# Stoffel-Labs/mpc-protocols

Hardware: AMD Instinct MI355X
Metric: shares/sec (compute_shares) + recons/sec (batch_recon), 256-bit Fr, 1/2/4/8 GPU (higher is better)
Workload: dtype u32; 1 GPU; compute_shares n=16 t=5 batch=2^20 secrets per GPU (BASELINE configs[1]); field=bls12-381 Fr, parallelism=batch-sharded x1, no data-path collective, field_impl=u29

## Files before the change

mpc-protocols_amd/csrc/kernels_mfma_bfly_ring.hpp:

```cpp
#pragma once
#include "bfly_ring_plan.hpp"
#include "kernels_mfma_bfly.hpp"

namespace hbmpc {
namespace mf {

HB_DEV void ring_dma16(const uint8_t* sbase, uint32_t voff, uint32_t lds_dst) {
    uint32_t keep;
    asm volatile("s_mov_b32 %0, m0\n\ts_mov_b32 m0, %3\n\ts_nop 4\n\tglobal_load_lds_dwordx4 %1, %2\n\ts_mov_b32 m0, %0"
                 : "=&s"(keep)
                 : "v"(voff), "s"(sbase), "s"(lds_dst)
                 : "memory");
}
using ring_flag_t = __attribute__((address_space(3))) volatile uint32_t;
HB_DEV uint32_t ring_flag(const ring_flag_t* p) { return __builtin_amdgcn_readfirstlane(*p); }

template <int M, int CW, int NP, int S, int D>
__global__ __launch_bounds__(64 * (CW + 1)) void k_mfma_bfly_ring(MfmaRowsArgs a) {
    static_assert(bfly_ring_shape_ok(M, NP, BflyRingShape{CW, S, D}), "ring shape");
    static_assert(M * (D - 1) <= 63, "vmcnt counts to 63");
    constexpr int ROWB = M * 1024 + MF_BFLY_BIAS;
    constexpr int NT = 64 * (CW + 1);
    constexpr int TILEB = M * 1024;
    extern __shared__ __attribute__((aligned(16))) uint8_t lds[];
    const int blk8 = (int)blockIdx.x >> 3;
    const uint32_t wg_in_role = (uint32_t)a.blk_idx[blk8] * 8 + (blockIdx.x & 7);
    const MfmaRole role = a.role[0];
    const uint32_t role_wgs = (uint32_t)a.role_nwg[0];
    bfly_table_to_lds<NT>(lds, a.table + (size_t)role.row0 * ROWB, NP * (ROWB / 16));
    uint8_t* const ring = lds + bfly_ring_table_bytes(M, NP);
    ring_flag_t* const filled = (ring_flag_t*)(lds + bfly_ring_flags_offset(M, NP, S));
    ring_flag_t* const freed = filled + S;
    if (threadIdx.x < 2 * S) filled[threadIdx.x] = 0;
    __syncthreads();
    const uint32_t lane = threadIdx.x & 63, wave = __builtin_amdgcn_readfirstlane(threadIdx.x >> 6);
    const uint32_t nitems = (uint32_t)bfly_ring_items(bfly_ring_ntiles(a.G), role_wgs, wg_in_role, CW);
    auto tile_of = [&](uint32_t q) { return bfly_ring_tile(role_wgs, wg_in_role, CW, q); };
    if (wave == CW) {
        if (nitems == 0) return;
        const size_t total = a.G * (size_t)(M * 32);
        auto wait_freed = [&](uint32_t q) {
            if (q >= S) {
                const uint32_t need = q / S;
                while (ring_flag(freed + q % S) != need) __builtin_amdgcn_s_sleep(1);
            }
        };
        auto publish = [&](uint32_t q) { filled[q % S] = q / S + 1; };
        auto piece = [&](size_t tb, int i) {
            const uint32_t off = (uint32_t)(i * 64 + lane) * 16u;
            const size_t left = total - tb;
            return left >= (size_t)TILEB || off + 16 <= left ? off : (uint32_t)(left - 16);
        };
        const uint32_t ring_lds = (uint32_t)(uintptr_t)ring;
        for (uint32_t q = 0; q < nitems; ++q) {
            wait_freed(q);
            const size_t tb = tile_of(q) * (size_t)(32 * M * 32);
            const uint32_t dst = __builtin_amdgcn_readfirstlane(ring_lds + (q % S) * TILEB);
#pragma unroll
            for (int i = 0; i < M; ++i) ring_dma16(a.in + tb, piece(tb, i), dst + i * 1024);
            if (q + 1 >= D) {
                asm volatile("s_waitcnt vmcnt(%0)" ::"n"(M * (D - 1)) : "memory");
                publish(q + 1 - D);
            }
        }
        asm volatile("s_waitcnt vmcnt(0)" ::: "memory");
        for (uint32_t q = nitems >= D - 1 ? nitems - (D - 1) : 0; q < nitems; ++q) publish(q);
        return;
    }
    const int c = lane & 31, h = lane >> 5;
    const Half H = make_half(h);
    for (uint32_t q = wave; q < nitems; q += CW) {
        const uint32_t slot = q % S, seq = q / S + 1;
        while (ring_flag(filled + slot) != seq) __builtin_amdgcn_s_sleep(1);
        asm volatile("" ::: "memory");
        v4i data[M];
        {
            const uint8_t* sp = ring + slot * TILEB + c * (M * 32) + 16 * h;
#pragma unroll
            for (int i = 0; i < M; ++i) data[i] = *reinterpret_cast<const v4i*>(sp + i * 32);
        }
        asm volatile("s_waitcnt lgkmcnt(0)" ::: "memory");
        freed[slot] = seq;
#pragma unroll
        for (int i = 0; i < M; ++i) data[i] = flip(data[i]);
        const BflyOut o = bfly_out(a, tile_of(q), c, h);
        auto store_row = [&](uint32_t k, bool exists, const uint32_t (&Rw)[4]) {
            uint8_t* qb = a.out_party_major ? a.out + (size_t)k * a.out_stride * 32 : a.out + (size_t)k * 32;
            if (exists && o.live) *reinterpret_cast<uint4*>(qb + o.qo) = make_uint4(Rw[0], Rw[1], Rw[2], Rw[3]);
        };
#pragma unroll
        for (int p = 0; p < NP; ++p) {
            uint32_t pe[8], pt[8];
            bfly_pair<M>(lds + (size_t)p * ROWB, lane, h, data, pe, pt);
            uint32_t k32 = (uint32_t)(role.row0 + p);
            asm volatile("" : "+s"(k32));
            {
                uint64_t T[4];
                uint32_t Rw[4];
#pragma unroll
                for (int j = 0; j < 4; ++j) T[j] = (uint64_t)(pe[2 * j + 1] + pt[2 * j + 1]) * H.k16 + (pe[2 * j] + pt[2 * j]);
                reduce_words(T, Rw, H);
                store_row(k32, true, Rw);
            }
            const bool partner = (int)k32 + a.half < a.nout;
            if (partner) {
                uint64_t T[4];
                uint32_t Rw[4];
#pragma unroll
                for (int j = 0; j < 4; ++j) T[j] = (uint64_t)(pe[2 * j + 1] - pt[2 * j + 1]) * H.k16 + (pe[2 * j] - pt[2 * j]);
                reduce_words(T, Rw, H);
                store_row(k32 + (uint32_t)a.half, true, Rw);
            }
        }
    }
}

}
}
```

mpc-protocols_amd/csrc/tu_mfma_bfly_ring.hip:

```cpp
#include <utility>

#include "kernels_mfma_bfly_ring.hpp"
#include "launchers.hpp"
namespace hbmpc {
namespace {
template <int M, int NP>
bool launch(const mf::MfmaRowsArgs& a, int device, hipStream_t s) {
    if constexpr (mf::bfly_ring_fits(M, NP)) {
        constexpr mf::BflyRingShape R = mf::BFLY_RING_LIB;
        const size_t lds = mf::bfly_ring_lds_bytes(M, NP, R.slots);
        static std::atomic<bool> attr_set[HBMPC_MAX_DEVICES];
        if (!ensure_dynamic_lds(reinterpret_cast<const void*>(&mf::k_mfma_bfly_ring<M, R.cw, NP, R.slots, R.depth>), attr_set, device, lds)) return false;
        hipLaunchKernelGGL((mf::k_mfma_bfly_ring<M, R.cw, NP, R.slots, R.depth>), dim3((unsigned)mf::mf_grid(a)), dim3(64 * (R.cw + 1)), lds, s, a);
        return true;
    }
    return false;
}
template <int M>
bool one(const mf::MfmaRowsArgs& a, int device, hipStream_t s) {
    if (a.role[0].nrows == 8) return launch<M, 8>(a, device, s);
    if (a.role[0].nrows == 4) return launch<M, 4>(a, device, s);
    return false;
}
template <int LO, int... I>
bool range(int m, const mf::MfmaRowsArgs& a, int device, hipStream_t s, std::integer_sequence<int, I...>) {
    bool hit = false;
    ((m == LO + I ? (hit = one<LO + I>(a, device, s)) : false), ...);
    return hit;
}
}
bool launch_mfma_bfly_ring(int m, const mf::MfmaRowsArgs& a, int device, hipStream_t s) {
    if (!a.in_chunk_major || a.in_b || a.ncoeffs || a.list_rows || a.other_stride || a.nroles != 1 || a.G == 0) return false;
    return range<2>(m, a, device, s, std::make_integer_sequence<int, mf::BFLY_RING_MAX_M - 1>{});
}
}
```

Baseline: 115.8 billion shares/s.

## Overlap ring prologue DMA with table load in butterfly ring kernel

The producer wave now issues its first D tile DMAs before the block barrier, while the compute waves load the twiddle table into LDS with direct global-to-LDS DMA instead of a cooperative copy. The flag init and __syncthreads now follow the table load, and the producer joins via s_barrier. This overlaps kernel startup latency (table load and first tile fetches) instead of serialising them. The block index indirection is dropped, and the launcher now rejects any non-identity blk_idx mapping. The producer no longer exits early when it has no items and always participates in the barrier.

```diff
diff --git a/mpc-protocols_amd/csrc/kernels_mfma_bfly_ring.hpp b/mpc-protocols_amd/csrc/kernels_mfma_bfly_ring.hpp
--- a/mpc-protocols_amd/csrc/kernels_mfma_bfly_ring.hpp
+++ b/mpc-protocols_amd/csrc/kernels_mfma_bfly_ring.hpp
@@ -20,24 +20,18 @@
     static_assert(bfly_ring_shape_ok(M, NP, BflyRingShape{CW, S, D}), "ring shape");
     static_assert(M * (D - 1) <= 63, "vmcnt counts to 63");
     constexpr int ROWB = M * 1024 + MF_BFLY_BIAS;
-    constexpr int NT = 64 * (CW + 1);
     constexpr int TILEB = M * 1024;
     extern __shared__ __attribute__((aligned(16))) uint8_t lds[];
-    const int blk8 = (int)blockIdx.x >> 3;
-    const uint32_t wg_in_role = (uint32_t)a.blk_idx[blk8] * 8 + (blockIdx.x & 7);
+    const uint32_t wg_in_role = blockIdx.x;
     const MfmaRole role = a.role[0];
     const uint32_t role_wgs = (uint32_t)a.role_nwg[0];
-    bfly_table_to_lds<NT>(lds, a.table + (size_t)role.row0 * ROWB, NP * (ROWB / 16));
     uint8_t* const ring = lds + bfly_ring_table_bytes(M, NP);
     ring_flag_t* const filled = (ring_flag_t*)(lds + bfly_ring_flags_offset(M, NP, S));
     ring_flag_t* const freed = filled + S;
-    if (threadIdx.x < 2 * S) filled[threadIdx.x] = 0;
-    __syncthreads();
     const uint32_t lane = threadIdx.x & 63, wave = __builtin_amdgcn_readfirstlane(threadIdx.x >> 6);
     const uint32_t nitems = (uint32_t)bfly_ring_items(bfly_ring_ntiles(a.G), role_wgs, wg_in_role, CW);
     auto tile_of = [&](uint32_t q) { return bfly_ring_tile(role_wgs, wg_in_role, CW, q); };
     if (wave == CW) {
-        if (nitems == 0) return;
         const size_t total = a.G * (size_t)(M * 32);
         auto wait_freed = [&](uint32_t q) {
             if (q >= S) {
@@ -52,21 +46,42 @@
             return left >= (size_t)TILEB || off + 16 <= left ? off : (uint32_t)(left - 16);
         };
         const uint32_t ring_lds = (uint32_t)(uintptr_t)ring;
-        for (uint32_t q = 0; q < nitems; ++q) {
-            wait_freed(q);
+        auto request = [&](uint32_t q) {
             const size_t tb = tile_of(q) * (size_t)(32 * M * 32);
             const uint32_t dst = __builtin_amdgcn_readfirstlane(ring_lds + (q % S) * TILEB);
 #pragma unroll
             for (int i = 0; i < M; ++i) ring_dma16(a.in + tb, piece(tb, i), dst + i * 1024);
-            if (q + 1 >= D) {
-                asm volatile("s_waitcnt vmcnt(%0)" ::"n"(M * (D - 1)) : "memory");
-                publish(q + 1 - D);
+        };
+#pragma unroll
+        for (int q = 0; q < D; ++q)
+            if ((uint32_t)q < nitems) request((uint32_t)q);
+        __builtin_amdgcn_s_barrier();
+        for (uint32_t q = D - 1; q < nitems; ++q) {
+            if (q >= D) {
+                wait_freed(q);
+                request(q);
             }
+            asm volatile("s_waitcnt vmcnt(%0)" ::"n"(M * (D - 1)) : "memory");
+            publish(q + 1 - D);
         }
         asm volatile("s_waitcnt vmcnt(0)" ::: "memory");
         for (uint32_t q = nitems >= D - 1 ? nitems - (D - 1) : 0; q < nitems; ++q) publish(q);
         return;
     }
+    {
+        static_assert(NP * ROWB % 1024 == 0, "the table is whole 1-KB pieces");
+        constexpr int KB = NP * ROWB / 1024;
+        const uint8_t* src = a.table + (size_t)role.row0 * ROWB;
+        const uint32_t lds0 = (uint32_t)(uintptr_t)lds;
+#pragma unroll
+        for (int j = 0; j < (KB + CW - 1) / CW; ++j) {
+            const uint32_t k = wave + (uint32_t)j * CW;
+            if (k < (uint32_t)KB) ring_dma16(src + (size_t)k * 1024, lane * 16u, __builtin_amdgcn_readfirstlane(lds0 + k * 1024));
+        }
+        asm volatile("s_waitcnt vmcnt(0)" ::: "memory");
+    }
+    if (threadIdx.x < 2 * S) filled[threadIdx.x] = 0;
+    __syncthreads();
     const int c = lane & 31, h = lane >> 5;
     const Half H = make_half(h);
     for (uint32_t q = wave; q < nitems; q += CW) {
diff --git a/mpc-protocols_amd/csrc/tu_mfma_bfly_ring.hip b/mpc-protocols_amd/csrc/tu_mfma_bfly_ring.hip
--- a/mpc-protocols_amd/csrc/tu_mfma_bfly_ring.hip
+++ b/mpc-protocols_amd/csrc/tu_mfma_bfly_ring.hip
@@ -31,6 +31,8 @@
 }
 bool launch_mfma_bfly_ring(int m, const mf::MfmaRowsArgs& a, int device, hipStream_t s) {
     if (!a.in_chunk_major || a.in_b || a.ncoeffs || a.list_rows || a.other_stride || a.nroles != 1 || a.G == 0) return false;
+    for (int j = 0; j < a.nblocks; ++j)
+        if (a.blk_idx[j] != j) return false;
     return range<2>(m, a, device, s, std::make_integer_sequence<int, mf::BFLY_RING_MAX_M - 1>{});
 }
 }
```

After: 116.8 billion shares/s, median of 6. About the same (+0.9%).

## Prefetch ring tiles before table load and use nontemporal output stores

Applied to the files above, without the earlier changes.

The loader wave now issues its first D tile DMAs before the block-wide barrier, so input fetch overlaps the coefficient table copy into LDS. Only the compute waves load the table, and they stage it through registers. The blk_idx byte is now read as a 32-bit word. Output stores switch to global_store_dwordx4 with the nt modifier by default, so the write-once share stream avoids polluting the cache. The risks are more complex barrier ordering (the loader returns only after the sync) and possible nt store penalties.

```diff
diff --git a/mpc-protocols_amd/csrc/kernels_mfma_bfly_ring.hpp b/mpc-protocols_amd/csrc/kernels_mfma_bfly_ring.hpp
--- a/mpc-protocols_amd/csrc/kernels_mfma_bfly_ring.hpp
+++ b/mpc-protocols_amd/csrc/kernels_mfma_bfly_ring.hpp
@@ -1,44 +1,72 @@
 #pragma once
+#include <stddef.h>
+
 #include "bfly_ring_plan.hpp"
 #include "kernels_mfma_bfly.hpp"
 
 namespace hbmpc {
 namespace mf {
 
+enum RingPolicy { RP_DEFAULT = 0, RP_NT = 1, RP_SC1 = 2, RP_SC0_SC1 = 3 };
+#define HBMPC_RING_DMA16(MOD)                                                                                                       \
+    asm volatile("s_mov_b32 %0, m0\n\ts_mov_b32 m0, %3\n\ts_nop 4\n\tglobal_load_lds_dwordx4 %1, %2" MOD "\n\ts_mov_b32 m0, %0" \
+                 : "=&s"(keep)                                                                                                      \
+                 : "v"(voff), "s"(sbase), "s"(lds_dst)                                                                              \
+                 : "memory")
+template <int POL = RP_DEFAULT>
 HB_DEV void ring_dma16(const uint8_t* sbase, uint32_t voff, uint32_t lds_dst) {
+    static_assert(POL == RP_DEFAULT || POL == RP_NT, "loader policy");
     uint32_t keep;
-    asm volatile("s_mov_b32 %0, m0\n\ts_mov_b32 m0, %3\n\ts_nop 4\n\tglobal_load_lds_dwordx4 %1, %2\n\ts_mov_b32 m0, %0"
-                 : "=&s"(keep)
-                 : "v"(voff), "s"(sbase), "s"(lds_dst)
-                 : "memory");
+    if constexpr (POL == RP_NT) HBMPC_RING_DMA16(" nt");
+    else HBMPC_RING_DMA16("");
 }
+#undef HBMPC_RING_DMA16
+template <int POL>
+HB_DEV void ring_store16(uint8_t* p, const uint32_t (&w)[4]) {
+    static_assert(POL == RP_NT || POL == RP_SC1 || POL == RP_SC0_SC1, "store policy");
+    const v4i v = {(int)w[0], (int)w[1], (int)w[2], (int)w[3]};
+    if constexpr (POL == RP_NT) asm volatile("global_store_dwordx4 %0, %1, off nt" ::"v"(p), "v"(v) : "memory");
+    else if constexpr (POL == RP_SC1) asm volatile("global_store_dwordx4 %0, %1, off sc1" ::"v"(p), "v"(v) : "memory");
+    else asm volatile("global_store_dwordx4 %0, %1, off sc0 sc1" ::"v"(p), "v"(v) : "memory");
+}
+constexpr int BFLY_RING_LOAD_POLICY = RP_DEFAULT, BFLY_RING_STORE_POLICY = RP_NT;
 using ring_flag_t = __attribute__((address_space(3))) volatile uint32_t;
 HB_DEV uint32_t ring_flag(const ring_flag_t* p) { return __builtin_amdgcn_readfirstlane(*p); }
 
-template <int M, int CW, int NP, int S, int D>
+template <int M, int CW, int NP, int S, int D, int LP = BFLY_RING_LOAD_POLICY, int SP = BFLY_RING_STORE_POLICY>
 __global__ __launch_bounds__(64 * (CW + 1)) void k_mfma_bfly_ring(MfmaRowsArgs a) {
     static_assert(bfly_ring_shape_ok(M, NP, BflyRingShape{CW, S, D}), "ring shape");
     static_assert(M * (D - 1) <= 63, "vmcnt counts to 63");
     constexpr int ROWB = M * 1024 + MF_BFLY_BIAS;
-    constexpr int NT = 64 * (CW + 1);
     constexpr int TILEB = M * 1024;
     extern __shared__ __attribute__((aligned(16))) uint8_t lds[];
     const int blk8 = (int)blockIdx.x >> 3;
-    const uint32_t wg_in_role = (uint32_t)a.blk_idx[blk8] * 8 + (blockIdx.x & 7);
+    static_assert(offsetof(MfmaRowsArgs, blk_idx) % 4 == 0, "blk_idx is read by words");
+    const uint32_t blk_word = reinterpret_cast<const uint32_t*>(a.blk_idx)[blk8 >> 2];
+    const uint32_t wg_in_role = ((blk_word >> (8 * (blk8 & 3))) & 0xffu) * 8 + (blockIdx.x & 7);
     const MfmaRole role = a.role[0];
     const uint32_t role_wgs = (uint32_t)a.role_nwg[0];
-    bfly_table_to_lds<NT>(lds, a.table + (size_t)role.row0 * ROWB, NP * (ROWB / 16));
     uint8_t* const ring = lds + bfly_ring_table_bytes(M, NP);
     ring_flag_t* const filled = (ring_flag_t*)(lds + bfly_ring_flags_offset(M, NP, S));
     ring_flag_t* const freed = filled + S;
-    if (threadIdx.x < 2 * S) filled[threadIdx.x] = 0;
-    __syncthreads();
     const uint32_t lane = threadIdx.x & 63, wave = __builtin_amdgcn_readfirstlane(threadIdx.x >> 6);
-    const uint32_t nitems = (uint32_t)bfly_ring_items(bfly_ring_ntiles(a.G), role_wgs, wg_in_role, CW);
+    auto items = [&] { return (uint32_t)bfly_ring_items(bfly_ring_ntiles(a.G), role_wgs, wg_in_role, CW); };
     auto tile_of = [&](uint32_t q) { return bfly_ring_tile(role_wgs, wg_in_role, CW, q); };
     if (wave == CW) {
-        if (nitems == 0) return;
+        const uint32_t nitems = items();
         const size_t total = a.G * (size_t)(M * 32);
+        auto piece = [&](size_t tb, int i) {
+            const uint32_t off = (uint32_t)(i * 64 + lane) * 16u;
+            const size_t left = total - tb;
+            return left >= (size_t)TILEB || off + 16 <= left ? off : (uint32_t)(left - 16);
+        };
+        const uint32_t ring_lds = (uint32_t)(uintptr_t)ring;
+        auto request = [&](uint32_t q) {
+            const size_t tb = tile_of(q) * (size_t)(32 * M * 32);
+            const uint32_t dst = __builtin_amdgcn_readfirstlane(ring_lds + (q % S) * TILEB);
+#pragma unroll
+            for (int i = 0; i < M; ++i) ring_dma16<LP>(a.in + tb, piece(tb, i), dst + i * 1024);
+        };
         auto wait_freed = [&](uint32_t q) {
             if (q >= S) {
                 const uint32_t need = q / S;
@@ -46,22 +74,18 @@
             }
         };
         auto publish = [&](uint32_t q) { filled[q % S] = q / S + 1; };
-        auto piece = [&](size_t tb, int i) {
-            const uint32_t off = (uint32_t)(i * 64 + lane) * 16u;
-            const size_t left = total - tb;
-            return left >= (size_t)TILEB || off + 16 <= left ? off : (uint32_t)(left - 16);
-        };
-        const uint32_t ring_lds = (uint32_t)(uintptr_t)ring;
-        for (uint32_t q = 0; q < nitems; ++q) {
+        for (uint32_t q = 0; q < nitems && q < (uint32_t)D; ++q) request(q);
+        __syncthreads();
+        if (nitems == 0) return;
+        if (nitems >= (uint32_t)D) {
+            asm volatile("s_waitcnt vmcnt(%0)" ::"n"(M * (D - 1)) : "memory");
+            publish(0);
+        }
+        for (uint32_t q = D; q < nitems; ++q) {
             wait_freed(q);
-            const size_t tb = tile_of(q) * (size_t)(32 * M * 32);
-            const uint32_t dst = __builtin_amdgcn_readfirstlane(ring_lds + (q % S) * TILEB);
-#pragma unroll
-            for (int i = 0; i < M; ++i) ring_dma16(a.in + tb, piece(tb, i), dst + i * 1024);
-            if (q + 1 >= D) {
-                asm volatile("s_waitcnt vmcnt(%0)" ::"n"(M * (D - 1)) : "memory");
-                publish(q + 1 - D);
-            }
+            request(q);
+            asm volatile("s_waitcnt vmcnt(%0)" ::"n"(M * (D - 1)) : "memory");
+            publish(q + 1 - D);
         }
         asm volatile("s_waitcnt vmcnt(0)" ::: "memory");
         for (uint32_t q = nitems >= D - 1 ? nitems - (D - 1) : 0; q < nitems; ++q) publish(q);
@@ -69,6 +93,27 @@
     }
     const int c = lane & 31, h = lane >> 5;
     const Half H = make_half(h);
+    uint32_t nitems;
+    {
+        constexpr int PIECES = NP * (ROWB / 16), NTC = 64 * CW, ROUNDS = (PIECES + NTC - 1) / NTC;
+        const uint8_t* src = a.table + (size_t)role.row0 * ROWB;
+        v4i t[ROUNDS];
+#pragma unroll
+        for (int k = 0; k < ROUNDS; ++k) {
+            const int p = (int)threadIdx.x + k * NTC;
+            t[k] = *reinterpret_cast<const v4i*>(src + (size_t)((k + 1) * NTC <= PIECES || p < PIECES ? p : PIECES - 1) * 16);
+        }
+        nitems = items();
+#pragma unroll
+        for (int k = 0; k < ROUNDS; ++k) asm volatile("" : "+v"(t[k]));
+#pragma unroll
+        for (int k = 0; k < ROUNDS; ++k) {
+            const int p = (int)threadIdx.x + k * NTC;
+            if ((k + 1) * NTC <= PIECES || p < PIECES) *reinterpret_cast<v4i*>(lds + (size_t)p * 16) = t[k];
+        }
+        if (threadIdx.x < 2 * S) filled[threadIdx.x] = 0;
+    }
+    __syncthreads();
     for (uint32_t q = wave; q < nitems; q += CW) {
         const uint32_t slot = q % S, seq = q / S + 1;
         while (ring_flag(filled + slot) != seq) __builtin_amdgcn_s_sleep(1);
@@ -86,7 +131,10 @@
         const BflyOut o = bfly_out(a, tile_of(q), c, h);
         auto store_row = [&](uint32_t k, bool exists, const uint32_t (&Rw)[4]) {
             uint8_t* qb = a.out_party_major ? a.out + (size_t)k * a.out_stride * 32 : a.out + (size_t)k * 32;
-            if (exists && o.live) *reinterpret_cast<uint4*>(qb + o.qo) = make_uint4(Rw[0], Rw[1], Rw[2], Rw[3]);
+            if (exists && o.live) {
+                if constexpr (SP == RP_DEFAULT) *reinterpret_cast<uint4*>(qb + o.qo) = make_uint4(Rw[0], Rw[1], Rw[2], Rw[3]);
+                else ring_store16<SP>(qb + o.qo, Rw);
+            }
         };
 #pragma unroll
         for (int p = 0; p < NP; ++p) {
```

New measurement: 118.0 billion shares/s before, 142.5 billion shares/s after, median of 6. 1.21x the previous value.
